# aosokin/os2d

Hardware: AMD Instinct MI355X
Metric: query-image-pairs/s (1280-px input, ResNet50, N-class) (higher is better)
Workload: dtype fftx3 (as fft; the per-bin complex GEMM on the fp16 MFMA with spectra split into fp16 hi+lo, 3 MFMAs per product, fp32 accumulate)

## Files before the change

### os2d_amd/csrc/spectra_pack.hip

```cpp
#include "tile_common.h"

namespace {

constexpr int SP_THR = 256;
constexpr int SP_KS = 7, SP_TAPS = 49, SP_R = 3;

struct cd {
  double re, im;
};

__device__ __forceinline__ cd sp_value(const double (&w)[SP_TAPS], const cd* __restrict__ tP, const cd* __restrict__ tQ, int u,
                                       int v, int P, int Q) {
  cd ep[SP_KS], eq[SP_KS];
#pragma unroll
  for (int t = 0; t < SP_KS; ++t) {
    const int pt = (SP_R - t + P) % P, ps = (SP_R - t + Q) % Q;
    ep[t] = tP[(u * pt) % P];
    eq[t] = tQ[(v * ps) % Q];
  }
  cd k{0.0, 0.0};
#pragma unroll
  for (int s = 0; s < SP_KS; ++s) {
    double rr = 0.0, ri = 0.0;
#pragma unroll
    for (int t = 0; t < SP_KS; ++t) {
      rr = fma(w[t * SP_KS + s], ep[t].re, rr);
      ri = fma(w[t * SP_KS + s], ep[t].im, ri);
    }
    k.re = fma(rr, eq[s].re, fma(-ri, eq[s].im, k.re));
    k.im = fma(rr, eq[s].im, fma(ri, eq[s].re, k.im));
  }
  return k;
}

template <int MODE>
__global__ __launch_bounds__(SP_THR) void spectra_pack_kernel(const double* __restrict__ wfold,
                                                              const double* __restrict__ twP, const double* __restrict__ twQ,
                                                              int C, int Cout, int P, int Q, int NBINS, int bins_per_block,
                                                              unsigned long long* __restrict__ amax, void* __restrict__ out,
                                                              float* __restrict__ wscale, int ufast) {
  extern __shared__ __attribute__((aligned(16))) unsigned char smem[];
  cd* tP = reinterpret_cast<cd*>(smem);
  cd* tQ = tP + P;
  const int tid = threadIdx.x, lane = tid & 63, wv = tid >> 6;
  for (int i = tid; i < P; i += SP_THR) tP[i] = cd{twP[2 * i], twP[2 * i + 1]};
  for (int i = tid; i < Q; i += SP_THR) tQ[i] = cd{twQ[2 * i], twQ[2 * i + 1]};
  __syncthreads();
  const int V = Q / 2 + 1, KSTEPS = (C + 7) / 8;
  const int cu = blockIdx.x % (KSTEPS * 2), half = blockIdx.x / (KSTEPS * 2);
  const int c4 = MODE == 1 ? (lane & 3) : wv;
  const int ol = MODE == 1 ? wv * 16 + (lane >> 2) : lane;
  const int c = cu * 4 + c4, o = half * 64 + ol;
  const bool live = c < C && o < Cout;
  double w[SP_TAPS];
#pragma unroll
  for (int k = 0; k < SP_TAPS; ++k) w[k] = live ? wfold[((size_t)o * C + c) * SP_TAPS + k] : 0.0;
  const int bin0 = blockIdx.y * bins_per_block, bin1 = min(bin0 + bins_per_block, NBINS);
  if (MODE == 0) {
    double m = 0.0;
    for (int bin = bin0; bin < min(bin1, P * V); ++bin) {
      const int u = ufast ? bin % P : bin / V, v = ufast ? bin / P : bin - u * V;
      const cd k = sp_value(w, tP, tQ, u, v, P, Q);
      m = fmax(m, fmax(fabs(k.re), fabs(k.im)));
    }
    if (live) atomicMax(amax + o, (unsigned long long)__double_as_longlong(m));
    return;
  }
  double scale = 1.0;
  if (MODE == 1) {
    const double mx = o < Cout ? __longlong_as_double((long long)amax[o]) : 0.0;
    int e = mx > 0.0 ? (int)floor(log2(32768.0 / mx)) : 0;
    e = max(-100, min(100, e));
    scale = ldexp(1.0, e);
    if (blockIdx.x % (KSTEPS * 2) == 0 && blockIdx.y == 0 && c4 == 0 && o < 128) wscale[o] = (float)ldexp(1.0, -e);
  }
  for (int bin = bin0; bin < bin1; ++bin) {
    cd k{0.0, 0.0};
    if (bin < P * V) {
      const int u = ufast ? bin % P : bin / V, v = ufast ? bin / P : bin - u * V;
      k = sp_value(w, tP, tQ, u, v, P, Q);
    }
    const int g = bin >> 3, j = bin & 7;
    if (MODE == 1) {
      const double vr = k.re * scale, vi = k.im * scale;
      const _Float16 hr = (_Float16)vr, hi_ = (_Float16)vi;
      const _Float16 lr = (_Float16)(vr - (double)hr), li = (_Float16)(vi - (double)hi_);
      const unsigned hbits = (unsigned)__builtin_bit_cast(unsigned short, hr) | ((unsigned)__builtin_bit_cast(unsigned short, hi_) << 16);
      const unsigned lbits = (unsigned)__builtin_bit_cast(unsigned short, lr) | ((unsigned)__builtin_bit_cast(unsigned short, li) << 16);
      const int ks = cu >> 1, grp = cu & 1;
      const size_t unit = ((((((size_t)g * 2 + half) * KSTEPS + ks) * 8 + j) * 2 + grp) * 2) * 64 + ol;
      unsigned* dst = reinterpret_cast<unsigned*>(out) + unit * 4 + c4;
      dst[0] = hbits;
      dst[64 * 4] = lbits;
    } else {
      if (c < C) {
        float2* dst = reinterpret_cast<float2*>(out) + ((((size_t)g * 2 + half) * C + c) * 8 + j) * 64 + ol;
        *dst = make_float2((float)k.re, (float)k.im);
      }
    }
  }
}

}

int os2d_launch_spectra_pack(const double* wfold, const double* twP64, const double* twQ64, int C, int Cout, int P, int Q,
                             int NBINS, int split, int u_fastest, void* out, void* workspace, hipStream_t stream) {
  const int V = Q / 2 + 1, KSTEPS = (C + 7) / 8;
  if (P * V > NBINS || (NBINS & 7) || Cout > 128 || P < 1 || Q < 2 || (Q & 1)) {
    os2d_set_error("spectra_pack: bad sizes (P=%d Q=%d NBINS=%d Cout=%d)", P, Q, NBINS, Cout);
    return -3;
  }
  const size_t lds = (size_t)(P + Q) * sizeof(cd);
  const int nb_y = 8, per = os2d_round_up((NBINS + nb_y - 1) / nb_y, 8);
  dim3 grid(2 * KSTEPS * 2, (NBINS + per - 1) / per);
  if (split) {
    unsigned long long* amax = static_cast<unsigned long long*>(workspace);
    hipError_t e = hipMemsetAsync(amax, 0, 128 * sizeof(unsigned long long), stream);
    if (e != hipSuccess) {
      os2d_set_error("hipMemsetAsync: %s", hipGetErrorString(e));
      return -4;
    }
    hipLaunchKernelGGL(spectra_pack_kernel<0>, grid, dim3(SP_THR), lds, stream, wfold, twP64, twQ64, C, Cout, P, Q, NBINS, per, amax,
                       nullptr, nullptr, u_fastest);
    int rc = os2d_launched("spectra_pack (row maxima)");
    if (rc) return rc;
    float* wscale = reinterpret_cast<float*>(static_cast<char*>(out) + (size_t)(NBINS / 8) * 2 * KSTEPS * 8 * 256 * 16);
    hipLaunchKernelGGL(spectra_pack_kernel<1>, grid, dim3(SP_THR), lds, stream, wfold, twP64, twQ64, C, Cout, P, Q, NBINS, per, amax,
                       out, wscale, u_fastest);
    return os2d_launched("spectra_pack (split)");
  }
  hipLaunchKernelGGL(spectra_pack_kernel<2>, grid, dim3(SP_THR), lds, stream, wfold, twP64, twQ64, C, Cout, P, Q, NBINS, per, nullptr,
                     out, nullptr, u_fastest);
  return os2d_launched("spectra_pack (complex64)");
}
```

### os2d_amd/csrc/spectral_f16.hip

```cpp
#include "tile_common.h"

namespace {


constexpr int SH_THR = 512;
constexpr int SH_WB = 4;
constexpr int SH_BINS = 8;
constexpr int SH_OH = 64, SH_NB = 64;
constexpr int SH_KC = 8;
constexpr int SH_STAGE = SH_WB * 2 * 2 * 64;
constexpr int SH_WSTAGE = 2 * SH_STAGE;
constexpr int SH_WRING = 2;

#define SH_MM(x_, y_, acc_) __builtin_amdgcn_mfma_f32_32x32x16_f16(x_, y_, acc_, 0, 0, 0)
__device__ __forceinline__ void sh_lds_barrier() { asm volatile("s_waitcnt lgkmcnt(0)\n\ts_barrier" ::: "memory"); }

template <bool XQ>
__global__ __launch_bounds__(SH_THR, 1) void spectral_gemm_f16_kernel(const u32x4* w16,
                                                                      const float* __restrict__ wscale,
                                                                      const f32x2* __restrict__ X,
                                                                      f32x2* __restrict__ Y,
                                                                      int NB, int C, int Cpad, int Cout, int NBINS, int G, float xscale,
                                                                      int nunits) {
  extern __shared__ __attribute__((aligned(16))) unsigned char smem[];
  u32x4* ldsW = reinterpret_cast<u32x4*>(smem);
  u32x4* ldsX = ldsW + SH_WRING * SH_WSTAGE;
  const int tid = threadIdx.x, lane = tid & 63, l31 = lane & 31, hw = lane >> 5;
  const int wv = __builtin_amdgcn_readfirstlane(tid >> 6);
  const int lidx = os2d_xcd_logical(blockIdx.x, gridDim.x);
  if (lidx >= nunits) return;
  constexpr int NBH = SH_BINS / SH_WB;
  const int bh = lidx % NBH, lg = lidx / NBH;
  const int nbt = (NB + SH_NB - 1) / SH_NB;
  const int bt = lg % nbt, g = lg / nbt;
  const int nb0 = bt * SH_NB, bin0 = g * SH_BINS + bh * SH_WB;
  const int KS = (C + SH_KC - 1) / SH_KC;
  const int ot = wv & 3, pt = wv >> 2;
  const int wq = wv & 3, wh = wv >> 2;

  f32x16 yr[SH_WB], yi[SH_WB];
#pragma unroll
  for (int j = 0; j < SH_WB; ++j)
#pragma unroll
    for (int r = 0; r < 16; ++r) {
      yr[j][r] = 0.f;
      yi[j][r] = 0.f;
    }

  const u32x4* wbase = w16 + ((size_t)(g * 2 + wh) * KS) * (SH_BINS * 256) + bh * SH_STAGE;
  u32x4 wra[4], wrb[4];
#define SH_LOAD_W(S, wr)                                                                                            \
  {                                                                                                                 \
    const u32x4* src_ = wbase + (size_t)(S) * (SH_BINS * 256);                                                      \
    _Pragma("unroll") for (int k_ = 0; k_ < 4; ++k_) wr[k_] = src_[(wq * 4 + k_) * 64 + lane];                      \
  }
#define SH_LOAD_W1(S, wr, K) wr[K] = (wbase + (size_t)(S) * (SH_BINS * 256))[(wq * 4 + (K)) * 64 + lane];
#define SH_STORE_W(S, wr)                                                                                           \
  {                                                                                                                 \
    _Pragma("unroll") for (int k_ = 0; k_ < 4; ++k_)                                                                \
        ldsW[((S) % SH_WRING) * SH_WSTAGE + wh * SH_STAGE + (wq * 4 + k_) * 64 + lane] = wr[k_];                    \
  }
  const int xn = XQ ? wv * 8 + (lane >> 3) : wq * 16 + (lane & 15);
  const int xj = XQ ? (lane & 1) : (lane >> 4) & 1, xg = XQ ? (lane >> 2) & 1 : lane >> 5;
  const int xwh = XQ ? (lane >> 1) & 1 : wh;
  const bool xn_ok = nb0 + xn < NB;
  const int nbl = min(SH_NB, NB - nb0);
  const size_t qblk = XQ ? (size_t)nb0 * (NBINS >> 2) + (size_t)(bin0 >> 2) * nbl : 0;
  const f32x2* xrow = XQ ? X + ((qblk + min(xn, nbl - 1)) * Cpad) * 4 + 2 * xj
                         : X + (size_t)min(nb0 + xn, NB - 1) * NBINS + bin0 + 2 * xj;
  const size_t xcs = XQ ? 4 : (size_t)NB * NBINS;
  u32x4 pfa[2], pfb[2];
#define SH_LOAD_X(S, pfx)                                                                                           \
  {                                                                                                                 \
    _Pragma("unroll") for (int i_ = 0; i_ < 2; ++i_) {                                                              \
      const int c_ = min((S)*SH_KC + xg * 4 + xwh * 2 + i_, C - 1);                                                 \
      pfx[i_] = *reinterpret_cast<const u32x4*>(xrow + (size_t)c_ * xcs);                                           \
    }                                                                                                               \
  }
#define SH_LOAD_X1(S, pfx, I)                                                                                       \
  {                                                                                                                 \
    const int c_ = min((S)*SH_KC + xg * 4 + xwh * 2 + (I), C - 1);                                                  \
    pfx[I] = *reinterpret_cast<const u32x4*>(xrow + (size_t)c_ * xcs);                                              \
  }
#define SH_STORE_X(S, pfx)                                                                                          \
  {                                                                                                                 \
    _Pragma("unroll") for (int b2_ = 0; b2_ < 2; ++b2_) {                                                           \
      f32x4 v4_;                                                                                                    \
      _Pragma("unroll") for (int i_ = 0; i_ < 2; ++i_) {                                                            \
        const bool ok_ = xn_ok && (S)*SH_KC + xg * 4 + xwh * 2 + i_ < C;                                            \
        _Pragma("unroll") for (int p_ = 0; p_ < 2; ++p_) {                                                          \
          const unsigned raw_ = pfx[i_][2 * b2_ + p_];    \
          v4_[2 * i_ + p_] = ok_ ? __uint_as_float(raw_) * xscale : 0.f;                                            \
        }                                                                                                           \
      }                                                                                                             \
      const half4 h_ = __builtin_convertvector(v4_, half4);                                                         \
      const u32x2 hp_ = __builtin_bit_cast(u32x2, h_);      \
      const u32x2 lp_ = {os2d_split_lo_pair(v4_[0], v4_[1], hp_[0]), os2d_split_lo_pair(v4_[2], v4_[3], hp_[1])};    \
      const half4 l_ = __builtin_bit_cast(half4, lp_);                                                              \
      char* dst_ = reinterpret_cast<char*>(ldsX + ((S)&1) * SH_STAGE + (((2 * xj + b2_) * 2 + xg) * 2) * 64 + xn) + xwh * 8; \
      *reinterpret_cast<half4*>(dst_) = h_;                    \
      *reinterpret_cast<half4*>(dst_ + 64 * 16) = l_;                                                               \
    }                                                                                                               \
  }
#define SH_REQUESTS_HOOK(SN, WN, PN, J)                                                                             \
  if ((J) == 0) {                                                                                                   \
    SH_LOAD_W1(SN, WN, 0)                                                                                           \
    SH_LOAD_W1(SN, WN, 1)                                                                                           \
    __builtin_amdgcn_sched_barrier(0);                                                                              \
  } else if ((J) == 1) {                                                                                            \
    SH_LOAD_W1(SN, WN, 2)                                                                                           \
    SH_LOAD_W1(SN, WN, 3)                                                                                           \
    __builtin_amdgcn_sched_barrier(0);                                                                              \
  } else if ((J) == 2) {                                                                                            \
    SH_LOAD_X1(SN, PN, 0)                                                                                           \
    SH_LOAD_X1(SN, PN, 1)                                                                                           \
    __builtin_amdgcn_sched_barrier(0);                                                                              \
  }
#define SH_COMPUTE(S, SN, WN, PN)                                                                                         \
  {                                                                                                                 \
                                         \
    const u32x4* aB = ldsW + ((S) % SH_WRING) * SH_WSTAGE + (ot >> 1) * SH_STAGE + (hw * 2) * 64 + (ot & 1) * 32 + l31; \
    const u32x4* bB = ldsX + ((S)&1) * SH_STAGE + (hw * 2) * 64 + pt * 32 + l31;                                    \
    half8 bq[2][2];                                                                                                 \
    u32x4 kq[2][2];                                                                                                 \
    bq[0][0] = *reinterpret_cast<const half8*>(bB);                                                                 \
    bq[0][1] = *reinterpret_cast<const half8*>(bB + 64);                                                            \
    kq[0][0] = aB[0];                                                                                               \
    kq[0][1] = aB[64];                                                                                              \
    _Pragma("unroll") for (int j = 0; j < SH_WB; ++j) {                                                             \
      if (j + 1 < SH_WB) {                                                                                          \
        bq[(j + 1) & 1][0] = *reinterpret_cast<const half8*>(bB + (j + 1) * 256);                                   \
        bq[(j + 1) & 1][1] = *reinterpret_cast<const half8*>(bB + (j + 1) * 256 + 64);                              \
        kq[(j + 1) & 1][0] = aB[(j + 1) * 256];                                                                     \
        kq[(j + 1) & 1][1] = aB[(j + 1) * 256 + 64];                                                                \
      }                                                                                                             \
      __builtin_amdgcn_sched_barrier(0);                                                                            \
      const half8 bhf = bq[j & 1][0], blf = bq[j & 1][1];                                                           \
      const u32x4 kh = kq[j & 1][0], kl = kq[j & 1][1];                       \
      u32x4 rh, rl, ih, il;                                                                                         \
      _Pragma("unroll") for (int d = 0; d < 4; ++d) {                                                               \
        rh[d] = kh[d] ^ 0x80000000u;                                                                 \
        rl[d] = kl[d] ^ 0x80000000u;                                                                                \
        ih[d] = __builtin_amdgcn_alignbit(kh[d], kh[d], 16);                                          \
        il[d] = __builtin_amdgcn_alignbit(kl[d], kl[d], 16);                                                        \
      }                                                                                                             \
      const half8 arh = __builtin_bit_cast(half8, rh), arl = __builtin_bit_cast(half8, rl);                         \
      const half8 aih = __builtin_bit_cast(half8, ih), ail = __builtin_bit_cast(half8, il);                         \
       \
      yr[j] = SH_MM(bhf, arl, yr[j]);                                                                               \
      yr[j] = SH_MM(blf, arh, yr[j]);                                                                               \
      yr[j] = SH_MM(bhf, arh, yr[j]);                                                                               \
      yi[j] = SH_MM(bhf, ail, yi[j]);                                                                               \
      yi[j] = SH_MM(blf, aih, yi[j]);                                                                               \
      yi[j] = SH_MM(bhf, aih, yi[j]);                                                                               \
      __builtin_amdgcn_sched_barrier(0);                                                                            \
      SH_REQUESTS_HOOK(SN, WN, PN, j)                                                                               \
    }                                                                                                               \
  }
#define SH_STEP(S, WC, PC, WN, PN)                                                                                  \
  {                                                                                                                 \
    const int sn_ = min((S) + 2, KS - 1);                                                                           \
    SH_COMPUTE(S, sn_, WN, PN)                                                                                      \
    __builtin_amdgcn_sched_barrier(0);                                                                              \
    SH_STORE_W((S) + 1, WC)                                                                                         \
    SH_STORE_X((S) + 1, PC)                                                                                         \
    sh_lds_barrier();                                                                                               \
  }
  SH_LOAD_W(0, wrb)
  SH_LOAD_X(0, pfb)
  SH_LOAD_W(min(1, KS - 1), wra)
  SH_LOAD_X(min(1, KS - 1), pfa)
  SH_STORE_W(0, wrb)
  SH_STORE_X(0, pfb)
  sh_lds_barrier();
  int s = 0;
  for (; s + 1 < KS; s += 2) {
    SH_STEP(s, wra, pfa, wrb, pfb)
    SH_STEP(s + 1, wrb, pfb, wra, pfa)
  }
  if (s < KS) SH_STEP(s, wra, pfa, wrb, pfb)
#undef SH_STEP
#undef SH_REQUESTS_HOOK
#undef SH_LOAD_W1
#undef SH_LOAD_X1
#undef SH_LOAD_W
#undef SH_STORE_W
#undef SH_COMPUTE
#undef SH_LOAD_X
#undef SH_STORE_X

  const float inv_x = 1.0f / xscale;
  const int o = ot * 32 + l31;
  if (o < Cout) {
    const float sc = wscale[o] * inv_x;
#pragma unroll
    for (int r = 0; r < 16; ++r) {
      const int nb = nb0 + pt * 32 + (r & 3) + 8 * (r >> 2) + 4 * hw;
      if (nb < NB) {
        float4* dst = XQ ? reinterpret_cast<float4*>(Y + ((qblk + (nb - nb0)) * Cout + o) * 4)
                         : reinterpret_cast<float4*>(Y + (((size_t)(bin0 >> 2) * NB + nb) * Cout + o) * 4);
        dst[0] = make_float4(yr[0][r] * sc, yi[0][r] * sc, yr[1][r] * sc, yi[1][r] * sc);
        dst[1] = make_float4(yr[2][r] * sc, yi[2][r] * sc, yr[3][r] * sc, yi[3][r] * sc);
      }
    }
  }
}

}

size_t os2d_spectral_weight16_size(int C, int NBINS) {
  const size_t KS = (size_t)(C + SH_KC - 1) / SH_KC;
  return (size_t)(NBINS / SH_BINS) * 2 * KS * SH_BINS * 256 * 16 + 128 * sizeof(float);
}

float os2d_spectral_xscale_for(int H, int W) {
  float s = 1.0f;
  while (s * 2.0f * (float)H * (float)W <= 65504.0f) s *= 2.0f;
  return s;
}

int os2d_launch_spectral_gemm_f16(const void* w16, const float* X, float* Y, int NB, int C, int Cout, int NBINS, float xscale,
                                  int x_quads, int Cpad, hipStream_t stream) {
  if (NBINS % SH_BINS || Cout > 2 * SH_OH) {
    os2d_set_error("spectral_gemm_f16: NBINS %d must be a multiple of %d and Cout %d <= %d", NBINS, SH_BINS, Cout, 2 * SH_OH);
    return -3;
  }
  const int G = NBINS / SH_BINS, nbt = (NB + SH_NB - 1) / SH_NB;
  const size_t lds = (size_t)(SH_WRING * SH_WSTAGE + 2 * SH_STAGE) * 16;
  if (x_quads && Cpad < C) {
    os2d_set_error("spectral_gemm_f16: channel stride %d < C %d", Cpad, C);
    return -1;
  }
  auto kern = x_quads ? spectral_gemm_f16_kernel<true> : spectral_gemm_f16_kernel<false>;
  if (int rc = os2d_set_dynamic_lds(kern, lds, "spectral_gemm_f16")) return rc;
  const long long units = (long long)G * nbt * (SH_BINS / SH_WB);
  const size_t KS = (size_t)(C + SH_KC - 1) / SH_KC;
  const float* wscale = reinterpret_cast<const float*>(static_cast<const char*>(w16) + (size_t)G * 2 * KS * SH_BINS * 256 * 16);
  unsigned grid;
  if (int rc = os2d_xcd_grid(units, "spectral_gemm_f16", &grid)) return rc;
  hipLaunchKernelGGL(kern, dim3(grid), dim3(SH_THR), lds, stream, static_cast<const u32x4*>(w16), wscale,
                     reinterpret_cast<const f32x2*>(X), reinterpret_cast<f32x2*>(Y), NB, C, Cpad, Cout, NBINS, G, xscale, (int)units);
  return os2d_launched("spectral_gemm_f16");
}
```

Measured before the change: 46130.

## Add narrow-Cout spectral GEMM shape that skips the idle output half

```diff
diff --git a/os2d_amd/csrc/spectra_pack.hip b/os2d_amd/csrc/spectra_pack.hip
--- a/os2d_amd/csrc/spectra_pack.hip
+++ b/os2d_amd/csrc/spectra_pack.hip
@@ -74,9 +74,10 @@
     scale = ldexp(1.0, e);
     if (blockIdx.x % (KSTEPS * 2) == 0 && blockIdx.y == 0 && c4 == 0 && o < 128) wscale[o] = (float)ldexp(1.0, -e);
   }
+  const bool narrow = MODE == 1 && Cout <= 64;
   for (int bin = bin0; bin < bin1; ++bin) {
     cd k{0.0, 0.0};
-    if (bin < P * V) {
+    if (bin < P * V && !(narrow && half)) {
       const int u = ufast ? bin % P : bin / V, v = ufast ? bin / P : bin - u * V;
       k = sp_value(w, tP, tQ, u, v, P, Q);
     }
@@ -88,7 +89,8 @@
       const unsigned hbits = (unsigned)__builtin_bit_cast(unsigned short, hr) | ((unsigned)__builtin_bit_cast(unsigned short, hi_) << 16);
       const unsigned lbits = (unsigned)__builtin_bit_cast(unsigned short, lr) | ((unsigned)__builtin_bit_cast(unsigned short, li) << 16);
       const int ks = cu >> 1, grp = cu & 1;
-      const size_t unit = ((((((size_t)g * 2 + half) * KSTEPS + ks) * 8 + j) * 2 + grp) * 2) * 64 + ol;
+      const size_t gh = narrow ? (size_t)half * (NBINS >> 3) + g : (size_t)g * 2 + half;
+      const size_t unit = ((((gh * KSTEPS + ks) * 8 + j) * 2 + grp) * 2) * 64 + ol;
       unsigned* dst = reinterpret_cast<unsigned*>(out) + unit * 4 + c4;
       dst[0] = hbits;
       dst[64 * 4] = lbits;
diff --git a/os2d_amd/csrc/spectral_f16.hip b/os2d_amd/csrc/spectral_f16.hip
--- a/os2d_amd/csrc/spectral_f16.hip
+++ b/os2d_amd/csrc/spectral_f16.hip
@@ -5,60 +5,72 @@
 
 constexpr int SH_THR = 512;
 constexpr int SH_WB = 4;
+constexpr int SH_NWB = 8;
 constexpr int SH_BINS = 8;
 constexpr int SH_OH = 64, SH_NB = 64;
 constexpr int SH_KC = 8;
-constexpr int SH_STAGE = SH_WB * 2 * 2 * 64;
-constexpr int SH_WSTAGE = 2 * SH_STAGE;
+constexpr int SH_BIN = 2 * 2 * 64;
 constexpr int SH_WRING = 2;
+
+template <int OW_, int WBG_>
+struct ShShape {
+  static constexpr int OW = OW_, WBG = WBG_;
+  static constexpr int BS = 2 / OW, JW = WBG / BS;
+  static constexpr int NBH = SH_BINS / WBG;
+  static constexpr int WSTAGE = OW * WBG * SH_BIN;
+  static constexpr int XSTAGE = WBG * SH_BIN;
+  static constexpr int NW = WSTAGE / SH_THR;
+  static constexpr int NXQ = WBG / 4;
+  static constexpr int NREQ = NW + 2 * NXQ;
+  static constexpr size_t lds_bytes = (size_t)(SH_WRING * WSTAGE + 2 * XSTAGE) * 16;
+  static_assert(JW == 2 || JW == 4, "a wave owns half a quad of bins or a whole one");
+  static_assert(NREQ <= 2 * JW, "two requests behind the matrix instructions of each bin");
+};
+using ShWide = ShShape<2, SH_WB>;
+using ShNarrow = ShShape<1, SH_NWB>;
+constexpr size_t SH_LDS_MAX = ShNarrow::lds_bytes > ShWide::lds_bytes ? ShNarrow::lds_bytes : ShWide::lds_bytes;
 
 #define SH_MM(x_, y_, acc_) __builtin_amdgcn_mfma_f32_32x32x16_f16(x_, y_, acc_, 0, 0, 0)
 __device__ __forceinline__ void sh_lds_barrier() { asm volatile("s_waitcnt lgkmcnt(0)\n\ts_barrier" ::: "memory"); }
 
-template <bool XQ>
-__global__ __launch_bounds__(SH_THR, 1) void spectral_gemm_f16_kernel(const u32x4* w16,
-                                                                      const float* __restrict__ wscale,
-                                                                      const f32x2* __restrict__ X,
-                                                                      f32x2* __restrict__ Y,
-                                                                      int NB, int C, int Cpad, int Cout, int NBINS, int G, float xscale,
-                                                                      int nunits) {
+template <bool XQ, class SH>
+__device__ __forceinline__ void sh_gemm_body(const u32x4* w16, const float* __restrict__ wscale, const f32x2* __restrict__ X,
+                                             f32x2* __restrict__ Y, int NB, int C, int Cpad, int Cout, int NBINS, float xscale,
+                                             int lidx) {
   extern __shared__ __attribute__((aligned(16))) unsigned char smem[];
   u32x4* ldsW = reinterpret_cast<u32x4*>(smem);
-  u32x4* ldsX = ldsW + SH_WRING * SH_WSTAGE;
+  u32x4* ldsX = ldsW + SH_WRING * SH::WSTAGE;
   const int tid = threadIdx.x, lane = tid & 63, l31 = lane & 31, hw = lane >> 5;
   const int wv = __builtin_amdgcn_readfirstlane(tid >> 6);
-  const int lidx = os2d_xcd_logical(blockIdx.x, gridDim.x);
-  if (lidx >= nunits) return;
-  constexpr int NBH = SH_BINS / SH_WB;
-  const int bh = lidx % NBH, lg = lidx / NBH;
+  const int bh = lidx % SH::NBH, lg = lidx / SH::NBH;
   const int nbt = (NB + SH_NB - 1) / SH_NB;
   const int bt = lg % nbt, g = lg / nbt;
-  const int nb0 = bt * SH_NB, bin0 = g * SH_BINS + bh * SH_WB;
+  const int nb0 = bt * SH_NB, bin0 = g * SH_BINS + bh * SH::WBG;
   const int KS = (C + SH_KC - 1) / SH_KC;
-  const int ot = wv & 3, pt = wv >> 2;
+  const int ot = wv & (2 * SH::OW - 1), pt = (wv / (2 * SH::OW)) & 1, bs = wv / (4 * SH::OW);
   const int wq = wv & 3, wh = wv >> 2;
 
-  f32x16 yr[SH_WB], yi[SH_WB];
+  f32x16 yr[SH::JW], yi[SH::JW];
 #pragma unroll
-  for (int j = 0; j < SH_WB; ++j)
+  for (int j = 0; j < SH::JW; ++j)
 #pragma unroll
     for (int r = 0; r < 16; ++r) {
       yr[j][r] = 0.f;
       yi[j][r] = 0.f;
     }
 
-  const u32x4* wbase = w16 + ((size_t)(g * 2 + wh) * KS) * (SH_BINS * 256) + bh * SH_STAGE;
-  u32x4 wra[4], wrb[4];
+  const u32x4* wbase = SH::OW == 2 ? w16 + ((size_t)(g * 2 + wh) * KS) * (SH_BINS * SH_BIN) + bh * (SH::WSTAGE / 2) + (wq * SH::NW) * 64
+                                   : w16 + ((size_t)g * KS) * (SH_BINS * SH_BIN) + bh * SH::WSTAGE + (wv * SH::NW) * 64;
+  u32x4 wra[SH::NW], wrb[SH::NW];
+#define SH_LOAD_W1(S, wr, K) wr[K] = (wbase + (size_t)(S) * (SH_BINS * SH_BIN))[(K) * 64 + lane];
 #define SH_LOAD_W(S, wr)                                                                                            \
   {                                                                                                                 \
-    const u32x4* src_ = wbase + (size_t)(S) * (SH_BINS * 256);                                                      \
-    _Pragma("unroll") for (int k_ = 0; k_ < 4; ++k_) wr[k_] = src_[(wq * 4 + k_) * 64 + lane];                      \
-  }
-#define SH_LOAD_W1(S, wr, K) wr[K] = (wbase + (size_t)(S) * (SH_BINS * 256))[(wq * 4 + (K)) * 64 + lane];
+    _Pragma("unroll") for (int k_ = 0; k_ < SH::NW; ++k_) SH_LOAD_W1(S, wr, k_)                                     \
+  }
 #define SH_STORE_W(S, wr)                                                                                           \
   {                                                                                                                 \
-    _Pragma("unroll") for (int k_ = 0; k_ < 4; ++k_)                                                                \
-        ldsW[((S) % SH_WRING) * SH_WSTAGE + wh * SH_STAGE + (wq * 4 + k_) * 64 + lane] = wr[k_];                    \
+    _Pragma("unroll") for (int k_ = 0; k_ < SH::NW; ++k_)                                                           \
+        ldsW[((S) % SH_WRING) * SH::WSTAGE + (wv * SH::NW + k_) * 64 + lane] = wr[k_];                              \
   }
   const int xn = XQ ? wv * 8 + (lane >> 3) : wq * 16 + (lane & 15);
   const int xj = XQ ? (lane & 1) : (lane >> 4) & 1, xg = XQ ? (lane >> 2) & 1 : lane >> 5;
@@ -69,27 +81,26 @@
   const f32x2* xrow = XQ ? X + ((qblk + min(xn, nbl - 1)) * Cpad) * 4 + 2 * xj
                          : X + (size_t)min(nb0 + xn, NB - 1) * NBINS + bin0 + 2 * xj;
   const size_t xcs = XQ ? 4 : (size_t)NB * NBINS;
-  u32x4 pfa[2], pfb[2];
+  const size_t xqs = XQ ? (size_t)nbl * Cpad * 4 : 4;
+  u32x4 pfa[2 * SH::NXQ], pfb[2 * SH::NXQ];
+#define SH_LOAD_X1(S, pfx, I)                                                                                       \
+  {                                                                                                                 \
+    const int c_ = min((S)*SH_KC + xg * 4 + xwh * 2 + ((I)&1), C - 1);                                              \
+    pfx[I] = *reinterpret_cast<const u32x4*>(xrow + ((I) >> 1) * xqs + (size_t)c_ * xcs);                           \
+  }
 #define SH_LOAD_X(S, pfx)                                                                                           \
   {                                                                                                                 \
-    _Pragma("unroll") for (int i_ = 0; i_ < 2; ++i_) {                                                              \
-      const int c_ = min((S)*SH_KC + xg * 4 + xwh * 2 + i_, C - 1);                                                 \
-      pfx[i_] = *reinterpret_cast<const u32x4*>(xrow + (size_t)c_ * xcs);                                           \
-    }                                                                                                               \
-  }
-#define SH_LOAD_X1(S, pfx, I)                                                                                       \
-  {                                                                                                                 \
-    const int c_ = min((S)*SH_KC + xg * 4 + xwh * 2 + (I), C - 1);                                                  \
-    pfx[I] = *reinterpret_cast<const u32x4*>(xrow + (size_t)c_ * xcs);                                              \
+    _Pragma("unroll") for (int i_ = 0; i_ < 2 * SH::NXQ; ++i_) SH_LOAD_X1(S, pfx, i_)                               \
   }
 #define SH_STORE_X(S, pfx)                                                                                          \
   {                                                                                                                 \
+    _Pragma("unroll") for (int q_ = 0; q_ < SH::NXQ; ++q_)                                                          \
     _Pragma("unroll") for (int b2_ = 0; b2_ < 2; ++b2_) {                                                           \
       f32x4 v4_;                                                                                                    \
       _Pragma("unroll") for (int i_ = 0; i_ < 2; ++i_) {                                                            \
         const bool ok_ = xn_ok && (S)*SH_KC + xg * 4 + xwh * 2 + i_ < C;                                            \
         _Pragma("unroll") for (int p_ = 0; p_ < 2; ++p_) {                                                          \
-          const unsigned raw_ = pfx[i_][2 * b2_ + p_];    \
+          const unsigned raw_ = pfx[2 * q_ + i_][2 * b2_ + p_];    \
           v4_[2 * i_ + p_] = ok_ ? __uint_as_float(raw_) * xscale : 0.f;                                            \
         }                                                                                                           \
       }                                                                                                             \
@@ -97,42 +108,40 @@
       const u32x2 hp_ = __builtin_bit_cast(u32x2, h_);      \
       const u32x2 lp_ = {os2d_split_lo_pair(v4_[0], v4_[1], hp_[0]), os2d_split_lo_pair(v4_[2], v4_[3], hp_[1])};    \
       const half4 l_ = __builtin_bit_cast(half4, lp_);                                                              \
-      char* dst_ = reinterpret_cast<char*>(ldsX + ((S)&1) * SH_STAGE + (((2 * xj + b2_) * 2 + xg) * 2) * 64 + xn) + xwh * 8; \
+      char* dst_ = reinterpret_cast<char*>(ldsX + ((S)&1) * SH::XSTAGE + (((4 * q_ + 2 * xj + b2_) * 2 + xg) * 2) * 64 + xn) + xwh * 8; \
       *reinterpret_cast<half4*>(dst_) = h_;                    \
       *reinterpret_cast<half4*>(dst_ + 64 * 16) = l_;                                                               \
     }                                                                                                               \
   }
 #define SH_REQUESTS_HOOK(SN, WN, PN, J)                                                                             \
-  if ((J) == 0) {                                                                                                   \
-    SH_LOAD_W1(SN, WN, 0)                                                                                           \
-    SH_LOAD_W1(SN, WN, 1)                                                                                           \
+  if (2 * (J) < SH::NREQ) {                                                                                         \
+    _Pragma("unroll") for (int r_ = 2 * (J); r_ < 2 * (J) + 2; ++r_) {                                              \
+      if (r_ < SH::NW) {                                                                                            \
+        SH_LOAD_W1(SN, WN, r_)                                                                                      \
+      } else if (r_ < SH::NREQ) {                                                                                   \
+        SH_LOAD_X1(SN, PN, r_ - SH::NW)                                                                             \
+      }                                                                                                             \
+    }                                                                                                               \
     __builtin_amdgcn_sched_barrier(0);                                                                              \
-  } else if ((J) == 1) {                                                                                            \
-    SH_LOAD_W1(SN, WN, 2)                                                                                           \
-    SH_LOAD_W1(SN, WN, 3)                                                                                           \
-    __builtin_amdgcn_sched_barrier(0);                                                                              \
-  } else if ((J) == 2) {                                                                                            \
-    SH_LOAD_X1(SN, PN, 0)                                                                                           \
-    SH_LOAD_X1(SN, PN, 1)                                                                                           \
-    __builtin_amdgcn_sched_barrier(0);                                                                              \
   }
 #define SH_COMPUTE(S, SN, WN, PN)                                                                                         \
   {                                                                                                                 \
-                                         \
-    const u32x4* aB = ldsW + ((S) % SH_WRING) * SH_WSTAGE + (ot >> 1) * SH_STAGE + (hw * 2) * 64 + (ot & 1) * 32 + l31; \
-    const u32x4* bB = ldsX + ((S)&1) * SH_STAGE + (hw * 2) * 64 + pt * 32 + l31;                                    \
+                     \
+    const u32x4* aB = ldsW + ((S) % SH_WRING) * SH::WSTAGE + (SH::OW == 2 ? (ot >> 1) * (SH::WSTAGE / 2) : bs * SH::JW * SH_BIN) + \
+                      (hw * 2) * 64 + (ot & 1) * 32 + l31;                                                          \
+    const u32x4* bB = ldsX + ((S)&1) * SH::XSTAGE + bs * SH::JW * SH_BIN + (hw * 2) * 64 + pt * 32 + l31;           \
     half8 bq[2][2];                                                                                                 \
     u32x4 kq[2][2];                                                                                                 \
     bq[0][0] = *reinterpret_cast<const half8*>(bB);                                                                 \
     bq[0][1] = *reinterpret_cast<const half8*>(bB + 64);                                                            \
     kq[0][0] = aB[0];                                                                                               \
     kq[0][1] = aB[64];                                                                                              \
-    _Pragma("unroll") for (int j = 0; j < SH_WB; ++j) {                                                             \
-      if (j + 1 < SH_WB) {                                                                                          \
-        bq[(j + 1) & 1][0] = *reinterpret_cast<const half8*>(bB + (j + 1) * 256);                                   \
-        bq[(j + 1) & 1][1] = *reinterpret_cast<const half8*>(bB + (j + 1) * 256 + 64);                              \
-        kq[(j + 1) & 1][0] = aB[(j + 1) * 256];                                                                     \
-        kq[(j + 1) & 1][1] = aB[(j + 1) * 256 + 64];                                                                \
+    _Pragma("unroll") for (int j = 0; j < SH::JW; ++j) {                                                            \
+      if (j + 1 < SH::JW) {                                                                                         \
+        bq[(j + 1) & 1][0] = *reinterpret_cast<const half8*>(bB + (j + 1) * SH_BIN);                                \
+        bq[(j + 1) & 1][1] = *reinterpret_cast<const half8*>(bB + (j + 1) * SH_BIN + 64);                           \
+        kq[(j + 1) & 1][0] = aB[(j + 1) * SH_BIN];                                                                  \
+        kq[(j + 1) & 1][1] = aB[(j + 1) * SH_BIN + 64];                                                             \
       }                                                                                                             \
       __builtin_amdgcn_sched_barrier(0);                                                                            \
       const half8 bhf = bq[j & 1][0], blf = bq[j & 1][1];                                                           \
@@ -191,27 +200,49 @@
 
   const float inv_x = 1.0f / xscale;
   const int o = ot * 32 + l31;
+  const int qw = (bs * SH::JW) >> 2;
   if (o < Cout) {
     const float sc = wscale[o] * inv_x;
 #pragma unroll
     for (int r = 0; r < 16; ++r) {
       const int nb = nb0 + pt * 32 + (r & 3) + 8 * (r >> 2) + 4 * hw;
       if (nb < NB) {
-        float4* dst = XQ ? reinterpret_cast<float4*>(Y + ((qblk + (nb - nb0)) * Cout + o) * 4)
-                         : reinterpret_cast<float4*>(Y + (((size_t)(bin0 >> 2) * NB + nb) * Cout + o) * 4);
-        dst[0] = make_float4(yr[0][r] * sc, yi[0][r] * sc, yr[1][r] * sc, yi[1][r] * sc);
-        dst[1] = make_float4(yr[2][r] * sc, yi[2][r] * sc, yr[3][r] * sc, yi[3][r] * sc);
+        float4* dst = XQ ? reinterpret_cast<float4*>(Y + ((qblk + (size_t)qw * nbl + (nb - nb0)) * Cout + o) * 4)
+                         : reinterpret_cast<float4*>(Y + (((size_t)((bin0 >> 2) + qw) * NB + nb) * Cout + o) * 4);
+        if (SH::JW == 4) {
+          dst[0] = make_float4(yr[0][r] * sc, yi[0][r] * sc, yr[1][r] * sc, yi[1][r] * sc);
+          dst[1] = make_float4(yr[SH::JW - 2][r] * sc, yi[SH::JW - 2][r] * sc, yr[SH::JW - 1][r] * sc, yi[SH::JW - 1][r] * sc);
+        } else {
+          dst[bs & 1] = make_float4(yr[0][r] * sc, yi[0][r] * sc, yr[1][r] * sc, yi[1][r] * sc);
+        }
       }
     }
   }
 }
 
-}
-
-size_t os2d_spectral_weight16_size(int C, int NBINS) {
+template <bool XQ>
+__global__ __launch_bounds__(SH_THR, 1) void spectral_gemm_f16_kernel(const u32x4* w16,
+                                                                      const float* __restrict__ wscale,
+                                                                      const f32x2* __restrict__ X,
+                                                                      f32x2* __restrict__ Y,
+                                                                      int NB, int C, int Cpad, int Cout, int NBINS, int G, float xscale,
+                                                                      int nunits) {
+  const int lidx = os2d_xcd_logical(blockIdx.x, gridDim.x);
+  if (lidx >= nunits) return;
+  if (Cout <= SH_OH)
+    sh_gemm_body<XQ, ShNarrow>(w16, wscale, X, Y, NB, C, Cpad, Cout, NBINS, xscale, lidx);
+  else
+    sh_gemm_body<XQ, ShWide>(w16, wscale, X, Y, NB, C, Cpad, Cout, NBINS, xscale, lidx);
+}
+
+}
+
+static size_t sh_scales_offset(int C, int NBINS) {
   const size_t KS = (size_t)(C + SH_KC - 1) / SH_KC;
-  return (size_t)(NBINS / SH_BINS) * 2 * KS * SH_BINS * 256 * 16 + 128 * sizeof(float);
-}
+  return (size_t)(NBINS / SH_BINS) * 2 * KS * SH_BINS * SH_BIN * 16;
+}
+
+size_t os2d_spectral_weight16_size(int C, int NBINS) { return sh_scales_offset(C, NBINS) + 128 * sizeof(float); }
 
 float os2d_spectral_xscale_for(int H, int W) {
   float s = 1.0f;
@@ -225,17 +256,17 @@
     os2d_set_error("spectral_gemm_f16: NBINS %d must be a multiple of %d and Cout %d <= %d", NBINS, SH_BINS, Cout, 2 * SH_OH);
     return -3;
   }
+  const bool narrow = Cout <= SH_OH;
   const int G = NBINS / SH_BINS, nbt = (NB + SH_NB - 1) / SH_NB;
-  const size_t lds = (size_t)(SH_WRING * SH_WSTAGE + 2 * SH_STAGE) * 16;
+  const size_t lds = narrow ? ShNarrow::lds_bytes : ShWide::lds_bytes;
   if (x_quads && Cpad < C) {
     os2d_set_error("spectral_gemm_f16: channel stride %d < C %d", Cpad, C);
     return -1;
   }
   auto kern = x_quads ? spectral_gemm_f16_kernel<true> : spectral_gemm_f16_kernel<false>;
-  if (int rc = os2d_set_dynamic_lds(kern, lds, "spectral_gemm_f16")) return rc;
-  const long long units = (long long)G * nbt * (SH_BINS / SH_WB);
-  const size_t KS = (size_t)(C + SH_KC - 1) / SH_KC;
-  const float* wscale = reinterpret_cast<const float*>(static_cast<const char*>(w16) + (size_t)G * 2 * KS * SH_BINS * 256 * 16);
+  if (int rc = os2d_set_dynamic_lds(kern, SH_LDS_MAX, "spectral_gemm_f16")) return rc;
+  const long long units = (long long)G * nbt * (narrow ? ShNarrow::NBH : ShWide::NBH);
+  const float* wscale = reinterpret_cast<const float*>(static_cast<const char*>(w16) + sh_scales_offset(C, NBINS));
   unsigned grid;
   if (int rc = os2d_xcd_grid(units, "spectral_gemm_f16", &grid)) return rc;
   hipLaunchKernelGGL(kern, dim3(grid), dim3(SH_THR), lds, stream, static_cast<const u32x4*>(w16), wscale,
```

Measured after the change: 47010, median of 6. 1.9% higher.

## Add 64-row output tile shape covering both bin quads per block when Cout fits

Applied to the files above, without the earlier changes.

```diff
diff --git a/os2d_amd/csrc/spectral_f16.hip b/os2d_amd/csrc/spectral_f16.hip
--- a/os2d_amd/csrc/spectral_f16.hip
+++ b/os2d_amd/csrc/spectral_f16.hip
@@ -1,3 +1,5 @@
+#include <stdlib.h>
+
 #include "tile_common.h"
 
 namespace {
@@ -15,27 +17,30 @@
 #define SH_MM(x_, y_, acc_) __builtin_amdgcn_mfma_f32_32x32x16_f16(x_, y_, acc_, 0, 0, 0)
 __device__ __forceinline__ void sh_lds_barrier() { asm volatile("s_waitcnt lgkmcnt(0)\n\ts_barrier" ::: "memory"); }
 
-template <bool XQ>
-__global__ __launch_bounds__(SH_THR, 1) void spectral_gemm_f16_kernel(const u32x4* w16,
-                                                                      const float* __restrict__ wscale,
-                                                                      const f32x2* __restrict__ X,
-                                                                      f32x2* __restrict__ Y,
-                                                                      int NB, int C, int Cpad, int Cout, int NBINS, int G, float xscale,
-                                                                      int nunits) {
+template <bool XQ, bool R64>
+__device__ __forceinline__ void spectral_gemm_f16_body(const u32x4* w16,
+                                                       const float* __restrict__ wscale,
+                                                       const f32x2* __restrict__ X,
+                                                       f32x2* __restrict__ Y,
+                                                       int NB, int C, int Cpad, int Cout, int NBINS, float xscale, int nunits) {
   extern __shared__ __attribute__((aligned(16))) unsigned char smem[];
   u32x4* ldsW = reinterpret_cast<u32x4*>(smem);
+  static_assert(XQ || !R64, "the 64-row shape reads spectra in quads of bins only");
+  constexpr int NQ = R64 ? 2 : 1;
+  constexpr int XSTAGE = NQ * SH_STAGE;
   u32x4* ldsX = ldsW + SH_WRING * SH_WSTAGE;
   const int tid = threadIdx.x, lane = tid & 63, l31 = lane & 31, hw = lane >> 5;
   const int wv = __builtin_amdgcn_readfirstlane(tid >> 6);
   const int lidx = os2d_xcd_logical(blockIdx.x, gridDim.x);
   if (lidx >= nunits) return;
-  constexpr int NBH = SH_BINS / SH_WB;
+  constexpr int NBH = SH_BINS / (SH_WB * NQ);
   const int bh = lidx % NBH, lg = lidx / NBH;
   const int nbt = (NB + SH_NB - 1) / SH_NB;
   const int bt = lg % nbt, g = lg / nbt;
   const int nb0 = bt * SH_NB, bin0 = g * SH_BINS + bh * SH_WB;
   const int KS = (C + SH_KC - 1) / SH_KC;
-  const int ot = wv & 3, pt = wv >> 2;
+  const int ot = R64 ? wv & 1 : wv & 3, pt = R64 ? (wv >> 1) & 1 : wv >> 2;
+  const int quad = R64 ? wv >> 2 : 0;
   const int wq = wv & 3, wh = wv >> 2;
 
   f32x16 yr[SH_WB], yi[SH_WB];
@@ -47,7 +52,7 @@
       yi[j][r] = 0.f;
     }
 
-  const u32x4* wbase = w16 + ((size_t)(g * 2 + wh) * KS) * (SH_BINS * 256) + bh * SH_STAGE;
+  const u32x4* wbase = w16 + ((size_t)(g * 2 + (R64 ? 0 : wh)) * KS) * (SH_BINS * 256) + (R64 ? wh : bh) * SH_STAGE;
   u32x4 wra[4], wrb[4];
 #define SH_LOAD_W(S, wr)                                                                                            \
   {                                                                                                                 \
@@ -69,27 +74,28 @@
   const f32x2* xrow = XQ ? X + ((qblk + min(xn, nbl - 1)) * Cpad) * 4 + 2 * xj
                          : X + (size_t)min(nb0 + xn, NB - 1) * NBINS + bin0 + 2 * xj;
   const size_t xcs = XQ ? 4 : (size_t)NB * NBINS;
-  u32x4 pfa[2], pfb[2];
+  const size_t xqs = R64 ? (size_t)nbl * Cpad * 4 : 0;
+  u32x4 pfa[2 * NQ], pfb[2 * NQ];
 #define SH_LOAD_X(S, pfx)                                                                                           \
   {                                                                                                                 \
-    _Pragma("unroll") for (int i_ = 0; i_ < 2; ++i_) {                                                              \
-      const int c_ = min((S)*SH_KC + xg * 4 + xwh * 2 + i_, C - 1);                                                 \
-      pfx[i_] = *reinterpret_cast<const u32x4*>(xrow + (size_t)c_ * xcs);                                           \
+    _Pragma("unroll") for (int i_ = 0; i_ < 2 * NQ; ++i_) {                                                         \
+      const int c_ = min((S)*SH_KC + xg * 4 + xwh * 2 + (R64 ? i_ & 1 : i_), C - 1);                                \
+      pfx[i_] = *reinterpret_cast<const u32x4*>(xrow + (R64 ? (i_ >> 1) * xqs : 0) + (size_t)c_ * xcs);             \
     }                                                                                                               \
   }
 #define SH_LOAD_X1(S, pfx, I)                                                                                       \
   {                                                                                                                 \
-    const int c_ = min((S)*SH_KC + xg * 4 + xwh * 2 + (I), C - 1);                                                  \
-    pfx[I] = *reinterpret_cast<const u32x4*>(xrow + (size_t)c_ * xcs);                                              \
-  }
-#define SH_STORE_X(S, pfx)                                                                                          \
+    const int c_ = min((S)*SH_KC + xg * 4 + xwh * 2 + ((I)&1), C - 1);                                              \
+    pfx[I] = *reinterpret_cast<const u32x4*>(xrow + (R64 ? ((I) >> 1) * xqs : 0) + (size_t)c_ * xcs);               \
+  }
+#define SH_STORE_XQ(S, pfx, q_)                                                                                     \
   {                                                                                                                 \
     _Pragma("unroll") for (int b2_ = 0; b2_ < 2; ++b2_) {                                                           \
       f32x4 v4_;                                                                                                    \
       _Pragma("unroll") for (int i_ = 0; i_ < 2; ++i_) {                                                            \
         const bool ok_ = xn_ok && (S)*SH_KC + xg * 4 + xwh * 2 + i_ < C;                                            \
         _Pragma("unroll") for (int p_ = 0; p_ < 2; ++p_) {                                                          \
-          const unsigned raw_ = pfx[i_][2 * b2_ + p_];    \
+          const unsigned raw_ = pfx[2 * q_ + i_][2 * b2_ + p_];    \
           v4_[2 * i_ + p_] = ok_ ? __uint_as_float(raw_) * xscale : 0.f;                                            \
         }                                                                                                           \
       }                                                                                                             \
@@ -97,10 +103,15 @@
       const u32x2 hp_ = __builtin_bit_cast(u32x2, h_);      \
       const u32x2 lp_ = {os2d_split_lo_pair(v4_[0], v4_[1], hp_[0]), os2d_split_lo_pair(v4_[2], v4_[3], hp_[1])};    \
       const half4 l_ = __builtin_bit_cast(half4, lp_);                                                              \
-      char* dst_ = reinterpret_cast<char*>(ldsX + ((S)&1) * SH_STAGE + (((2 * xj + b2_) * 2 + xg) * 2) * 64 + xn) + xwh * 8; \
+      char* dst_ = reinterpret_cast<char*>(ldsX + ((S)&1) * XSTAGE + q_ * SH_STAGE + (((2 * xj + b2_) * 2 + xg) * 2) * 64 + xn) + xwh * 8; \
       *reinterpret_cast<half4*>(dst_) = h_;                    \
       *reinterpret_cast<half4*>(dst_ + 64 * 16) = l_;                                                               \
     }                                                                                                               \
+  }
+#define SH_STORE_X(S, pfx)                                                                                          \
+  {                                                                                                                 \
+    SH_STORE_XQ(S, pfx, 0)                                                                                          \
+    if constexpr (R64) SH_STORE_XQ(S, pfx, 1)                                                                       \
   }
 #define SH_REQUESTS_HOOK(SN, WN, PN, J)                                                                             \
   if ((J) == 0) {                                                                                                   \
@@ -115,12 +126,16 @@
     SH_LOAD_X1(SN, PN, 0)                                                                                           \
     SH_LOAD_X1(SN, PN, 1)                                                                                           \
     __builtin_amdgcn_sched_barrier(0);                                                                              \
+  } else if (R64) {                                                                                                 \
+    SH_LOAD_X1(SN, PN, 2 * (NQ - 1))                                                                                \
+    SH_LOAD_X1(SN, PN, 2 * (NQ - 1) + 1)                                                                            \
+    __builtin_amdgcn_sched_barrier(0);                                                                              \
   }
 #define SH_COMPUTE(S, SN, WN, PN)                                                                                         \
   {                                                                                                                 \
                                          \
-    const u32x4* aB = ldsW + ((S) % SH_WRING) * SH_WSTAGE + (ot >> 1) * SH_STAGE + (hw * 2) * 64 + (ot & 1) * 32 + l31; \
-    const u32x4* bB = ldsX + ((S)&1) * SH_STAGE + (hw * 2) * 64 + pt * 32 + l31;                                    \
+    const u32x4* aB = ldsW + ((S) % SH_WRING) * SH_WSTAGE + (R64 ? quad : ot >> 1) * SH_STAGE + (hw * 2) * 64 + (ot & 1) * 32 + l31; \
+    const u32x4* bB = ldsX + ((S)&1) * XSTAGE + quad * SH_STAGE + (hw * 2) * 64 + pt * 32 + l31;                    \
     half8 bq[2][2];                                                                                                 \
     u32x4 kq[2][2];                                                                                                 \
     bq[0][0] = *reinterpret_cast<const half8*>(bB);                                                                 \
@@ -188,6 +203,7 @@
 #undef SH_COMPUTE
 #undef SH_LOAD_X
 #undef SH_STORE_X
+#undef SH_STORE_XQ
 
   const float inv_x = 1.0f / xscale;
   const int o = ot * 32 + l31;
@@ -197,7 +213,7 @@
     for (int r = 0; r < 16; ++r) {
       const int nb = nb0 + pt * 32 + (r & 3) + 8 * (r >> 2) + 4 * hw;
       if (nb < NB) {
-        float4* dst = XQ ? reinterpret_cast<float4*>(Y + ((qblk + (nb - nb0)) * Cout + o) * 4)
+        float4* dst = XQ ? reinterpret_cast<float4*>(Y + ((qblk + (size_t)quad * nbl + (nb - nb0)) * Cout + o) * 4)
                          : reinterpret_cast<float4*>(Y + (((size_t)(bin0 >> 2) * NB + nb) * Cout + o) * 4);
         dst[0] = make_float4(yr[0][r] * sc, yi[0][r] * sc, yr[1][r] * sc, yi[1][r] * sc);
         dst[1] = make_float4(yr[2][r] * sc, yi[2][r] * sc, yr[3][r] * sc, yi[3][r] * sc);
@@ -206,6 +222,20 @@
   }
 }
 
+template <bool XQ>
+__global__ __launch_bounds__(SH_THR, 1) void spectral_gemm_f16_kernel(const u32x4* w16, const float* __restrict__ wscale,
+                                                                      const f32x2* __restrict__ X, f32x2* __restrict__ Y, int NB, int C,
+                                                                      int Cpad, int Cout, int NBINS, int rows64, float xscale,
+                                                                      int nunits) {
+  if constexpr (XQ) {
+    if (rows64) {
+      spectral_gemm_f16_body<true, true>(w16, wscale, X, Y, NB, C, Cpad, Cout, NBINS, xscale, nunits);
+      return;
+    }
+  }
+  spectral_gemm_f16_body<XQ, false>(w16, wscale, X, Y, NB, C, Cpad, Cout, NBINS, xscale, nunits);
+}
+
 }
 
 size_t os2d_spectral_weight16_size(int C, int NBINS) {
@@ -225,20 +255,25 @@
     os2d_set_error("spectral_gemm_f16: NBINS %d must be a multiple of %d and Cout %d <= %d", NBINS, SH_BINS, Cout, 2 * SH_OH);
     return -3;
   }
+  static const bool rows64_env = [] {
+    const char* e = getenv("OS2D_GEMM_ROWS64");
+    return !(e && e[0] == '0');
+  }();
+  const bool rows64 = x_quads && Cout <= SH_OH && rows64_env;
   const int G = NBINS / SH_BINS, nbt = (NB + SH_NB - 1) / SH_NB;
-  const size_t lds = (size_t)(SH_WRING * SH_WSTAGE + 2 * SH_STAGE) * 16;
+  const size_t lds = (size_t)(SH_WRING * SH_WSTAGE + 2 * (rows64 ? 2 : 1) * SH_STAGE) * 16;
   if (x_quads && Cpad < C) {
     os2d_set_error("spectral_gemm_f16: channel stride %d < C %d", Cpad, C);
     return -1;
   }
   auto kern = x_quads ? spectral_gemm_f16_kernel<true> : spectral_gemm_f16_kernel<false>;
   if (int rc = os2d_set_dynamic_lds(kern, lds, "spectral_gemm_f16")) return rc;
-  const long long units = (long long)G * nbt * (SH_BINS / SH_WB);
+  const long long units = (long long)G * nbt * (rows64 ? 1 : SH_BINS / SH_WB);
   const size_t KS = (size_t)(C + SH_KC - 1) / SH_KC;
   const float* wscale = reinterpret_cast<const float*>(static_cast<const char*>(w16) + (size_t)G * 2 * KS * SH_BINS * 256 * 16);
   unsigned grid;
   if (int rc = os2d_xcd_grid(units, "spectral_gemm_f16", &grid)) return rc;
   hipLaunchKernelGGL(kern, dim3(grid), dim3(SH_THR), lds, stream, static_cast<const u32x4*>(w16), wscale,
-                     reinterpret_cast<const f32x2*>(X), reinterpret_cast<f32x2*>(Y), NB, C, Cpad, Cout, NBINS, G, xscale, (int)units);
+                     reinterpret_cast<const f32x2*>(X), reinterpret_cast<f32x2*>(Y), NB, C, Cpad, Cout, NBINS, (int)rows64, xscale, (int)units);
   return os2d_launched("spectral_gemm_f16");
 }
```

After: 49350 before, 50090 after, median of 6. 1.5% higher.
